# mspaintenjoyer/DepthEstimation

Measured on AMD Instinct MI355X. Metric: disparity Mpix/s at 1080p d_max=128; 1/2/4/8-GPU scaling + %HBM roofline, higher is better.
Workload: dtype u8

## Files before the change

depthestimation_amd/csrc/dsx_bm.hip:

```cpp
#include "dsx_internal.h"
#include "dsx_partition.h"
#include "dsx_subpix.h"

constexpr int kWpe = 3;
constexpr int kWpeSsd = 4;

#ifndef DSX_ROWSTEP_PAIRTAIL
#define DSX_ROWSTEP_PAIRTAIL 0
#endif
#ifndef DSX_ROWSTEP_DIVQ
#define DSX_ROWSTEP_DIVQ 1
#endif
#ifndef DSX_ROWSTEP_OVERLAP
#define DSX_ROWSTEP_OVERLAP 1
#endif
#ifndef DSX_ROWSTEP_AHEAD
#define DSX_ROWSTEP_AHEAD 1
#endif
#ifndef DSX_ROWSTEP_SREF
#define DSX_ROWSTEP_SREF 0
#endif
#ifndef DSX_ROWSTEP_SARGS
#define DSX_ROWSTEP_SARGS DSX_ROWSTEP_SREF
#endif
#ifndef DSX_ROWSTEP_STAGEAHEAD
#define DSX_ROWSTEP_STAGEAHEAD 0
#endif
constexpr bool kRowstepStageahead = DSX_ROWSTEP_STAGEAHEAD;
#ifndef DSX_ROWSTEP_STORELATE
#define DSX_ROWSTEP_STORELATE 1
#endif
constexpr bool kRowstepStorelate = DSX_ROWSTEP_STORELATE;
constexpr bool kRowstepSref = DSX_ROWSTEP_SREF;
constexpr bool kRowstepSargs = DSX_ROWSTEP_SARGS;
constexpr bool kRowstepOverlap = DSX_ROWSTEP_OVERLAP;
constexpr bool kRowstepAhead = DSX_ROWSTEP_AHEAD;
constexpr bool kRowstepPairtail = DSX_ROWSTEP_PAIRTAIL;
constexpr bool kRowstepDivq = DSX_ROWSTEP_DIVQ;
#ifndef DSX_ROWSTEP_ATID
#define DSX_ROWSTEP_ATID 1
#endif
#ifndef DSX_ROWSTEP_KEY2
#define DSX_ROWSTEP_KEY2 1
#endif
#ifndef DSX_ROWSTEP_MERGE
#define DSX_ROWSTEP_MERGE 1
#endif
constexpr bool kRowstepMerge = DSX_ROWSTEP_MERGE;
constexpr bool kRowstepAtid = DSX_ROWSTEP_ATID;
constexpr bool kRowstepKey2 = DSX_ROWSTEP_KEY2;
#ifndef DSX_SEGSTART_AHEAD
#define DSX_SEGSTART_AHEAD 1
#endif
#ifndef DSX_SEGSTART_BATCH
#define DSX_SEGSTART_BATCH 1
#endif
#ifndef DSX_SEGSTART_SPART
#define DSX_SEGSTART_SPART 0
#endif
#ifndef DSX_SEGSTART_ROW0
#define DSX_SEGSTART_ROW0 0
#endif
constexpr bool kSegstartRow0 = DSX_SEGSTART_ROW0;
constexpr bool kSegstartAhead = DSX_SEGSTART_AHEAD;
constexpr bool kSegstartBatch = DSX_SEGSTART_BATCH;
constexpr bool kSegstartSpart = DSX_SEGSTART_SPART;

#include <algorithm>
#include <cstdio>
#include <cstdlib>
#include <cstring>
#include <mutex>
#include <type_traits>
#include <utility>
#include <vector>

namespace dsx {

typedef unsigned short u16x2 __attribute__((ext_vector_type(2)));
typedef uint32_t u32x2 __attribute__((ext_vector_type(2)));
__device__ __forceinline__ u32x2 lds_read_b64(const uint8_t *p) {
    return *(const volatile __attribute__((address_space(3))) u32x2 *)p;
}

__device__ __forceinline__ u16x2 as2(uint32_t v) { return __builtin_bit_cast(u16x2, v); }
__device__ __forceinline__ uint32_t as1(u16x2 v) { return __builtin_bit_cast(uint32_t, v); }
__device__ __forceinline__ int clampi2(int v, int lo, int hi) { return v < lo ? lo : (v > hi ? hi : v); }
__device__ __forceinline__ uint32_t umin2(uint32_t a, uint32_t b) { return a < b ? a : b; }
__device__ __forceinline__ u16x2 add_sub2(u16x2 a, u16x2 p, u16x2 q) { return as2(as1(a) + as1(p) - as1(q)); }
__device__ __forceinline__ int mad_i24(int a, int b, int c) {
    int r;
    asm("v_mad_i32_i24 %0, %1, %2, %3" : "=v"(r) : "v"(a), "v"(b), "v"(c));
    return r;
}
__device__ __forceinline__ uint32_t sad_hi_u8(uint32_t a, uint32_t b, uint32_t c) {
    return __builtin_amdgcn_sad_hi_u8(a, b, c);
}
__device__ __forceinline__ uint32_t min_shr1(uint32_t src, uint32_t key) {
    asm("s_nop 1\n\tv_min_u32_dpp %0, %1, %0 wave_shr:1 row_mask:0xf bank_mask:0xf" : "+v"(key) : "v"(src));
    return key;
}
#pragma clang diagnostic push
#pragma clang diagnostic ignored "-Winline-asm"
template <int OFF0, int STRIDE>
__device__ __forceinline__ void lds_store8_addtid(uint32_t m0base, const uint32_t (&v)[8]) {
    static_assert(OFF0 >= 0 && OFF0 + 7 * STRIDE < 65536, "16-bit offset field");
    asm volatile("s_mov_b32 m0, %8\n\ts_nop 0\n\t"
                 "ds_write_addtid_b32 %0 offset:%9\n\t"
                 "ds_write_addtid_b32 %1 offset:%10\n\t"
                 "ds_write_addtid_b32 %2 offset:%11\n\t"
                 "ds_write_addtid_b32 %3 offset:%12\n\t"
                 "ds_write_addtid_b32 %4 offset:%13\n\t"
                 "ds_write_addtid_b32 %5 offset:%14\n\t"
                 "ds_write_addtid_b32 %6 offset:%15\n\t"
                 "ds_write_addtid_b32 %7 offset:%16"
                 :
                 : "v"(v[0]), "v"(v[1]), "v"(v[2]), "v"(v[3]), "v"(v[4]), "v"(v[5]), "v"(v[6]), "v"(v[7]), "s"(m0base),
                   "n"(OFF0), "n"(OFF0 + STRIDE), "n"(OFF0 + 2 * STRIDE), "n"(OFF0 + 3 * STRIDE), "n"(OFF0 + 4 * STRIDE),
                   "n"(OFF0 + 5 * STRIDE), "n"(OFF0 + 6 * STRIDE), "n"(OFF0 + 7 * STRIDE)
                 : "memory", "m0");
}
#pragma clang diagnostic pop
__device__ __forceinline__ void lds_drain() { asm volatile("s_waitcnt lgkmcnt(0)" ::: "memory"); }
__device__ __forceinline__ uint32_t lds_offset(const uint8_t *p) {
    return (uint32_t)(uintptr_t)(const __attribute__((address_space(3))) uint8_t *)p;
}
__host__ __device__ constexpr int rnd16(int v) { return (v + 15) & ~15; }
template <int R, bool SSD, int NW>
struct Geo {
    static constexpr int TX = 32;
    static constexpr int NC = TX + 2 * R;
    static constexpr int KD = SSD ? 1 : 2;
    static constexpr int LDW = 64 * KD;
    static constexpr int Dp = NW * LDW;
    static constexpr int NT = 64 * NW;
    static constexpr int TPP = NT / TX;
    static constexpr int DSL = Dp / TPP;
    static constexpr int CB = SSD ? 4 : 2;
    static constexpr int PITCH = Dp * CB + 16;
    static constexpr int NJ = NC + Dp;
    static constexpr int REFW = rnd16(NC + 4);
    static constexpr int SROW = rnd16(NJ * 4 + 16);
    static constexpr int MAXJ = (NJ + NT - 1) / NT;
    static constexpr int NB = DSL / 8;
    static constexpr int REFB = rnd16(4 * (NC + 8));
    static constexpr int SLOT = SROW + REFB;
    static constexpr int SMEM0 = 4 * SLOT + TX * PITCH;
    static constexpr int SMEM = SMEM0 > (2 * R + 1) * SLOT ? SMEM0 : (2 * R + 1) * SLOT;
    static constexpr int XRB = 128;
};

#ifdef DSX_STAMPS
#define DSX_STAMP(i)                                                                        \
    do {                                                                                    \
        __builtin_amdgcn_sched_barrier(0);                                                  \
        uint64_t t_;                                                                        \
        asm volatile("s_memtime %0\n\ts_waitcnt lgkmcnt(0)" : "=s"(t_)::"memory");          \
        __builtin_amdgcn_sched_barrier(0);                                                  \
        if ((i) > 0) ph[(i)-1] += t_ - t_prev;                                              \
        t_prev = t_;                                                                        \
    } while (0)
#else
#define DSX_STAMP(i) \
    do {             \
    } while (0)
#endif

__device__ __forceinline__ void lds_barrier() {
    __builtin_amdgcn_fence(__ATOMIC_RELEASE, "workgroup", "local");
    __builtin_amdgcn_s_barrier();
    __builtin_amdgcn_fence(__ATOMIC_ACQUIRE, "workgroup", "local");
}

template <int NW>
__device__ __forceinline__ void block_sync() {
    if constexpr (NW == 1) {
        __builtin_amdgcn_fence(__ATOMIC_ACQ_REL, "wavefront", "local");
    } else {
        lds_barrier();
    }
}

template <int TPP>
__device__ __forceinline__ uint32_t gmin(uint32_t v) {
    if constexpr (TPP > 1) v = umin2(v, (uint32_t)__builtin_amdgcn_update_dpp(0, (int)v, 0xB1, 0xF, 0xF, false));
    if constexpr (TPP > 2) v = umin2(v, (uint32_t)__builtin_amdgcn_update_dpp(0, (int)v, 0x4E, 0xF, 0xF, false));
    if constexpr (TPP > 4) v = umin2(v, (uint32_t)__builtin_amdgcn_ds_swizzle((int)v, 0x101F));
    if constexpr (TPP > 8) v = umin2(v, (uint32_t)__builtin_amdgcn_ds_swizzle((int)v, 0x201F));
    return v;
}


typedef const __attribute__((address_space(4))) uint32_t cu32;
typedef const __attribute__((address_space(1))) uint8_t gu8;
typedef const __attribute__((address_space(1))) uint32_t gu32;
typedef __attribute__((address_space(1))) uint8_t gw8;
typedef __attribute__((address_space(1))) int16_t g16;
typedef __attribute__((address_space(1))) float gf32;

template <bool RELOAD>
__device__ __forceinline__ Bm2Args kargs_row(const Bm2Args &a) {
    if constexpr (RELOAD) {
        typedef __attribute__((address_space(4))) const Bm2Args KArgs;
        KArgs *p = (KArgs *)__builtin_amdgcn_kernarg_segment_ptr();
        asm volatile("" : "+s"(p));
        return *(const Bm2Args *)p;
    } else {
        return a;
    }
}

template <int R, bool SSD, int NW, int SIDE, bool FAST, bool ABS, bool LRFULL>
__device__ __forceinline__ void bm2_segment(const Bm2Args &a_in, uint8_t *smem, int x0, int yb, int ye, long fin, long fout,
                                            bool lr_on, int done0, const int (&pe)[3], int &qcur, int wvu
#ifdef DSX_STAMPS
                                            , uint64_t (&ph)[8], uint64_t &t_prev, uint64_t &nsteps
#endif
) {
    using G = Geo<R, SSD, NW>;
    constexpr int TX = G::TX, NC = G::NC, Dp = G::Dp, NT = G::NT, TPP = G::TPP, DSL = G::DSL, CB = G::CB,
                  PITCH = G::PITCH, NJ = G::NJ, SLOT = G::SLOT, NB = G::NB, NJ4 = (NJ + 3) / 4;
    constexpr int side = SIDE;
    const Bm2Args a = kargs_row<SIDE == 3>(a_in);
    constexpr bool FSS = SSD && !ABS && R <= 5 && (SIDE == 0 || SIDE == 3 || SIDE == 4);
    constexpr bool SGK = SIDE == 4;
    constexpr uint32_t OFF = FSS ? 0x4B000000u : 0u;
    constexpr int CW = (!FSS && (SSD || SIDE == 3)) ? 4 : 8, NCH = (NC + CW - 1) / CW;
    typedef typename std::conditional<FSS, float, typename std::conditional<SSD, uint32_t, u16x2>::type>::type acc_t;
    uint8_t *tile = smem + 4 * SLOT;

    constexpr bool LANE_RB = SSD && !ABS && NW >= 4;
    int ln = 0;
    if constexpr (LANE_RB)
        asm volatile("v_mbcnt_lo_u32_b32 %0, -1, 0\n\tv_mbcnt_hi_u32_b32 %0, -1, %0" : "=v"(ln));
    else
        ln = (int)threadIdx.x & 63;
    const int tid = LANE_RB ? (wvu << 6) + ln : (int)threadIdx.x;
    const int wv = LANE_RB ? wvu : tid >> 6;
    const int H = a.H, W = a.W, m = a.m, D = a.D;
    const int64_t stride = a.stride;
    const int d0 = SSD ? (wv * 64 + ln) : (wv * 128 + 2 * ln);
    const uint32_t padv = a.padv;
    const int PB = side == 1 ? (x0 - R + m) : (x0 - R - m + NC - 1);
    const int sgn = side == 1 ? 1 : -1;

    constexpr int NC4 = (NC + 3) / 4;
    constexpr bool RL2 = !SSD;
    uint32_t ofs_r = (uint32_t)(x0 - R + 4 * min(tid, NC4 - 1));
    uint32_t ofs_s = side == 1 ? (uint32_t)(PB + 4 * min(tid, NJ4 - 1)) : (uint32_t)(PB - 4 * min(tid, NJ4 - 1) - 3);
    constexpr bool MRG = kRowstepMerge && RL2 && FAST && SIDE != 3 && SIDE != 2 && !(SIDE == 4 && R >= 7);
    static_assert(!MRG || NJ4 + NC4 <= NT, "merged staging: a lane per staged dword");
    const bool m_s = tid < NJ4;
    const int m_r = min(tid - NJ4, NC4 - 1);
    const uint8_t *m_base = m_s ? a.src + fin + ofs_s : a.ref + fin + (uint32_t)(x0 - R + 4 * m_r);
    const bool m_dn = m_s && side != 1;
    const uint32_t m_sel0 = m_dn ? 0x0C0C0C03u : 0x0C0C0C00u, m_sel1 = m_dn ? 0x0C0C0C02u : 0x0C0C0C01u,
                   m_sel2 = m_dn ? 0x0C0C0C01u : 0x0C0C0C02u, m_sel3 = m_dn ? 0x0C0C0C00u : 0x0C0C0C03u;
    const uint32_t m_lane = m_s ? (uint32_t)(16 * tid) : (uint32_t)(G::SROW + 16 * m_r);
    auto ldm = [&](int r, uint32_t &w) __attribute__((always_inline)) {
        const int yy = clampi2(r, 0, H - 1);
        long ro = (long)yy * stride;
        asm("" : "+s"(ro));
        w = *reinterpret_cast<const uint32_t *>(m_base + ro);
    };
    auto stm = [&](uint8_t *sp, uint32_t w) __attribute__((always_inline)) {
        if (tid < NJ4 + NC4)
            *reinterpret_cast<uint4 *>(sp) = make_uint4(__builtin_amdgcn_perm(0u, w, m_sel0), __builtin_amdgcn_perm(0u, w, m_sel1),
                                                        __builtin_amdgcn_perm(0u, w, m_sel2), __builtin_amdgcn_perm(0u, w, m_sel3));
    };
    constexpr bool SR0 = kSegstartRow0 && kSegstartBatch && MRG && R <= 4 && (SIDE == 0 || SIDE == 4);
    uint32_t sr_n = 0, sr_o = 0;
    auto ld = [&](int r, uint32_t &w0, uint32_t &w1, uint32_t &w2, uint32_t &w3, uint32_t &rf) __attribute__((always_inline)) {
        const int yy = clampi2(r, 0, H - 1);
        const uint8_t *srow_ = a.src + fin + (long)yy * stride;
        const uint8_t *rrow_ = a.ref + fin + (long)yy * stride;
        if constexpr (RL2) {
            asm("" : "+s"(srow_));
            asm("" : "+s"(rrow_));
        }
        typedef typename std::conditional<RL2, gu8, const uint8_t>::type row8;
        typedef typename std::conditional<RL2, gu32, const uint32_t>::type row32;
        typedef typename std::conditional<RL2, uint32_t, int>::type rix;
        row8 *srow = (row8 *)srow_, *rrow = (row8 *)rrow_;
        const int tr = min(tid, NC4 - 1);
        if constexpr (FAST) {
            if constexpr (RL2) {
                rf = *reinterpret_cast<row32 *>(rrow + ofs_r);
            } else {
                rf = *reinterpret_cast<row32 *>(rrow + x0 - R + 4 * tr);
            }
        } else {
            uint32_t v = 0;
#pragma unroll
            for (int q = 0; q < 4; ++q) v |= (uint32_t)rrow[(rix)clampi2(x0 - R + 4 * tr + q, 0, W - 1)] << (8 * q);
            rf = v;
        }
        if constexpr (FAST) {
            const int tj = min(tid, NJ4 - 1);
            row8 *p;
            if constexpr (RL2) {
                p = srow + ofs_s;
            } else {
                p = side == 1 ? srow + PB + 4 * tj : (SIDE == 3 && NW == 1) ? srow + (PB - 4 * tj - 3) : srow + PB - 4 * tj - 3;
            }
            w0 = *reinterpret_cast<row32 *>(p);
            if constexpr (RL2) w1 = w2 = w3 = 0;
        } else {
            uint32_t v[4];
            int t4 = 4 * tid;
            if constexpr (!SSD && NW == 1 && SIDE == 3)
                asm volatile("" : "+v"(t4));
#pragma unroll
            for (int q = 0; q < 4; ++q) {
                const int j = min(t4 + q, NJ - 1);
                const int pp = PB + sgn * j;
                uint32_t t = srow[(rix)clampi2(pp, 0, W - 1)];
                if constexpr (FSS) t = __float_as_uint((float)t);
                v[q] = t;
            }
            w0 = v[0];
            w1 = v[1];
            w2 = v[2];
            w3 = v[3];
        }
    };
    auto st = [&](int sl, uint32_t w0, uint32_t w1, uint32_t w2, uint32_t w3, uint32_t rf) __attribute__((always_inline)) {
        if (FSS && tid < NC4) {
            *reinterpret_cast<uint4 *>(smem + sl * SLOT + G::SROW + 16 * tid) =
                make_uint4(__float_as_uint((float)(rf & 0xFFu)), __float_as_uint((float)((rf >> 8) & 0xFFu)),
                           __float_as_uint((float)((rf >> 16) & 0xFFu)), __float_as_uint((float)(rf >> 24)));
        } else if (tid < NC4) {
            *reinterpret_cast<uint4 *>(smem + sl * SLOT + G::SROW + 16 * tid) =
                make_uint4(rf & 0xFFu, (rf >> 8) & 0xFFu, (rf >> 16) & 0xFFu, rf >> 24);
        }
        if constexpr (FAST) {
            const uint32_t dw = w0;
            if (side == 1) {
                w0 = dw & 0xFFu; w1 = (dw >> 8) & 0xFFu; w2 = (dw >> 16) & 0xFFu; w3 = dw >> 24;
            } else if constexpr (FSS) {
                w0 = __float_as_uint((float)(dw >> 24)); w1 = __float_as_uint((float)((dw >> 16) & 0xFFu));
                w2 = __float_as_uint((float)((dw >> 8) & 0xFFu)); w3 = __float_as_uint((float)(dw & 0xFFu));
            } else {
                w0 = dw >> 24; w1 = (dw >> 16) & 0xFFu; w2 = (dw >> 8) & 0xFFu; w3 = dw & 0xFFu;
            }
        }
        if (tid < NJ4) *reinterpret_cast<uint4 *>(smem + sl * SLOT + 16 * tid) = make_uint4(w0, w1, w2, w3);
    };
    auto st_at = [&](uint8_t *sp, uint32_t w0, uint32_t w1, uint32_t w2, uint32_t w3, uint32_t rf) __attribute__((always_inline)) {
        if (tid < NC4)
            *reinterpret_cast<uint4 *>(sp + G::SROW) = make_uint4(rf & 0xFFu, (rf >> 8) & 0xFFu, (rf >> 16) & 0xFFu, rf >> 24);
        if constexpr (FAST) {
// ... 174 lines not shown
        uint32_t ae[NC], ao[NC];
#pragma unroll
        for (int c = 0; c < NC; ++c) ae[c] = ao[c] = 0;
        constexpr bool IAH = kSegstartAhead && R <= 5;
        if constexpr (IAH) {
#pragma unroll 1
            for (int g = 0; g < NGR; ++g) {
                uint32_t rv[2][4], p0[2][4], p1[2][4];
                auto ird = [&](auto qc) __attribute__((always_inline)) {
                    constexpr int q = decltype(qc)::value, c0 = 4 * q, t = q & 1;
                    const uint4 rr = *reinterpret_cast<const uint4 *>(smem + NGR * TPG + g * RG + 4 * c0);
                    rv[t][0] = rr.x; rv[t][1] = rr.y; rv[t][2] = rr.z; rv[t][3] = rr.w;
#pragma unroll
                    for (int c = 0; c < 4; ++c) {
                        if (c0 + c < NC) {
                            if constexpr (ABS) {
                                p0[t][c] = *reinterpret_cast<const uint32_t *>(tb + g * TPG + (NC - 1 - c0 - c) * 8);
                            } else {
                                const uint2 pr = *reinterpret_cast<const uint2 *>(tb + g * TPG + (NC - 1 - c0 - c) * 8);
                                p0[t][c] = pr.x;
                                p1[t][c] = pr.y;
                            }
                        }
                    }
                };
                auto isad = [&](auto qc) __attribute__((always_inline)) {
                    constexpr int q = decltype(qc)::value, c0 = 4 * q, t = q & 1;
#pragma unroll
                    for (int c = 0; c < 4; ++c) {
                        if (c0 + c < NC) {
                            ae[c0 + c] = __builtin_amdgcn_sad_u8(rv[t][c], p0[t][c], ae[c0 + c]);
                            if constexpr (!ABS) ao[c0 + c] = __builtin_amdgcn_sad_u8(rv[t][c], p1[t][c], ao[c0 + c]);
                        }
                    }
                };
                auto ichunk = [&](auto qc) __attribute__((always_inline)) {
                    constexpr int q = decltype(qc)::value;
                    if constexpr (q < NC4) {
                        __builtin_amdgcn_sched_barrier(0);
                        if constexpr (q + 1 < NC4) ird(std::integral_constant<int, q + 1>{});
                        __builtin_amdgcn_sched_barrier(0);
                        isad(qc);
                    }
                };
                ird(std::integral_constant<int, 0>{});
                ichunk(std::integral_constant<int, 0>{}); ichunk(std::integral_constant<int, 1>{});
                ichunk(std::integral_constant<int, 2>{}); ichunk(std::integral_constant<int, 3>{});
                ichunk(std::integral_constant<int, 4>{}); ichunk(std::integral_constant<int, 5>{});
                ichunk(std::integral_constant<int, 6>{}); ichunk(std::integral_constant<int, 7>{});
                ichunk(std::integral_constant<int, 8>{}); ichunk(std::integral_constant<int, 9>{});
                ichunk(std::integral_constant<int, 10>{}); ichunk(std::integral_constant<int, 11>{});
                static_assert(NC4 <= 12, "column chunks of the transposed init");
                __builtin_amdgcn_sched_barrier(0);
            }
        } else {
#pragma unroll 1
        for (int g = 0; g < NGR; ++g) {
#pragma unroll
            for (int q = 0; q < NC4; ++q) {
                const int c0 = 4 * q;
                const uint4 rr = *reinterpret_cast<const uint4 *>(smem + NGR * TPG + g * RG + 4 * c0);
                const uint32_t rv[4] = {rr.x, rr.y, rr.z, rr.w};
#pragma unroll
                for (int c = 0; c < 4; ++c) {
                    if (c0 + c < NC) {
                        if constexpr (ABS) {
                            const uint32_t p0 = *reinterpret_cast<const uint32_t *>(tb + g * TPG + (NC - 1 - c0 - c) * 8);
                            ae[c0 + c] = __builtin_amdgcn_sad_u8(rv[c], p0, ae[c0 + c]);
                        } else {
                            const uint2 pr = *reinterpret_cast<const uint2 *>(tb + g * TPG + (NC - 1 - c0 - c) * 8);
                            ae[c0 + c] = __builtin_amdgcn_sad_u8(rv[c], pr.x, ae[c0 + c]);
                            ao[c0 + c] = __builtin_amdgcn_sad_u8(rv[c], pr.y, ao[c0 + c]);
                        }
                    }
                }
            }
        }
        }
#pragma unroll
        for (int c = 0; c < NC; ++c) {
            if constexpr (ABS) cs[c] = ae[c];
            else cs[c] = as2(ae[c] | (ao[c] << 16));
        }
        }

    } else {
    block_sync<NW>();
    {
        constexpr int IG = 3;
#pragma unroll 1
        for (int i0 = 0; i0 <= 2 * R; i0 += IG) {
            uint32_t iw[IG][5];
#pragma unroll
            for (int i = 0; i < IG; ++i)
                if (i0 + i <= 2 * R) ld(yb - R + i0 + i, iw[i][0], iw[i][1], iw[i][2], iw[i][3], iw[i][4]);
#pragma unroll
            for (int i = 0; i < IG; ++i)
                if (i0 + i <= 2 * R) st(i0 + i, iw[i][0], iw[i][1], iw[i][2], iw[i][3], iw[i][4]);
        }
    }
    block_sync<NW>();
#pragma unroll 1
    for (int i = 0; i <= 2 * R; ++i) {
        uint32_t nx = 0;
#pragma unroll
        for (int q = 0; q < NCH; ++q) {
            const int c0 = CW * q;
            uint32_t sw[CW + 1], rw[CW];
            float rf8[8];
            s_chunk(i, c0, sw, nx);
            if constexpr (FSS) ref_chunkf(i, c0, rf8);
            else ref_chunk(i, c0, rw);
#pragma unroll
            for (int c = 0; c < CW; ++c) {
                if (c0 + c < NC) {
                    if constexpr (FSS) {
                        const float t = rf8[c] - __uint_as_float(sw[c]);
                        cs[c0 + c] = __builtin_fmaf(t, t, cs[c0 + c]);
                    } else if constexpr (ABS) {
                        cs[c0 + c] = __builtin_amdgcn_sad_u16(rw[c], sw[c], cs[c0 + c]);
                    } else if constexpr (SSD) {
                        const int t = (int)rw[c] - (int)sw[c];
                        cs[c0 + c] += (uint32_t)__mul24(t, t);
                    } else {
                        cs[c0 + c] = as2(sad_hi_u8(rw[c], pair_e1(sw, c), __builtin_amdgcn_sad_u8(rw[c], pair_e0(sw, c), as1(cs[c0 + c]))));
                    }
                }
            }
            if constexpr (SSD) __builtin_amdgcn_sched_barrier(0);
        }
    }
    }
    block_sync<NW>();

    for (int q = tid; q < TX * (Dp - D); q += NT) {
        const int k = q / (Dp - D), d = D + (q - k * (Dp - D));
        if constexpr (SSD) *reinterpret_cast<uint32_t *>(tile + k * PITCH + d * 4) = padv + OFF;
        else *reinterpret_cast<uint16_t *>(tile + k * PITCH + d * 2) = (uint16_t)padv;
    }
    block_sync<NW>();

    const bool edge = side == 1 && (x0 + m < 0 || x0 + TX - 1 + m + Dp - 1 > W - 1);
    const bool dodd = !SSD && (D & 1);
    const bool lane_writes = d0 < D;

    uint32_t stg = (MRG ? m_lane : (uint32_t)(16 * tid)) + (uint32_t)((2 - (yb & 1) * 2) * SLOT);
    constexpr bool PTAIL = kRowstepPairtail && !SSD && SIDE == 0 && NW == 1;
    constexpr bool DIVQ = kRowstepDivq && !SSD && SIDE == 0;
    uint32_t kp0 = 0, kp1 = 0;
    constexpr bool CUQ = !SSD && SIDE == 0 && NW == 1 && R < 6 && kRowstepKey2 && !PTAIL;
    constexpr bool OVL = kRowstepOverlap && CUQ, AHD = kRowstepAhead && CUQ;
    constexpr bool STA = kRowstepStageahead && OVL;
    constexpr bool STL = kRowstepStorelate && OVL;
    int e_fx = 0;
    float e_pf = 0.0f;
    constexpr int CQ = 4, NQ = (NC + CQ - 1) / CQ;
    constexpr bool SREF = kRowstepSref && CUQ && FAST && OVL && R < 5;
    constexpr bool SRA = kRowstepSargs && CUQ && OVL && R < 5;
    static_assert(!SREF || NQ == NC4, "one reference dword per column chunk");
    uint32_t qn[NC4 + 1] = {}, qo[NC4 + 1] = {}, shn = 0, sho = 0;
    auto sld = [&](int r, uint32_t(&q)[NC4 + 1], uint32_t &sh) __attribute__((always_inline)) {
        const int yy = clampi2(r, 0, H - 1);
        const uintptr_t p = (uintptr_t)(a.ref + fin + (long)yy * stride + (x0 - R));
        typedef const __attribute__((address_space(4))) uint8_t cu8;
        cu8 *b = (cu8 *)(p & ~(uintptr_t)3);
#pragma unroll
        for (int i = 0; i < NC4; ++i) q[i] = *(cu32 *)(b + 4 * i);
        q[NC4] = *(cu32 *)(b + ((((uint32_t)p + 4u * NC4 - 1u) & ~3u) - ((uint32_t)p & ~3u)));
        sh = ((uint32_t)p & 3u) * 8u;
    };
    auto sbyte = [](uint32_t w, int c) __attribute__((always_inline)) -> uint32_t {
        return c == 3 ? w >> 24 : (w >> (8 * c)) & 0xFFu;
    };
    constexpr int RPS = NQ >= 10 ? 1 : 2, NRS = 8 / RPS;
    static_assert(NQ >= NRS + 2, "a column chunk per stage up to the element keys");
    const int ek = tid / TPP, eh = tid % TPP, ex = x0 + ek;
    const uint8_t *epx = tile + ek * PITCH + eh * DSL * CB;
    uint4 etv[2] = {};
    uint32_t ekmin = 0, ecb = 0, egblk = 0, ecm = 0, ecp = 0;
    int eb = 0, ef = 0, eden = 1;
    bool esp = false;
    auto emin8 = [](uint4 v) __attribute__((always_inline)) -> uint32_t {
        const u16x2 mm = __builtin_elementwise_min(__builtin_elementwise_min(as2(v.x), as2(v.y)),
                                                   __builtin_elementwise_min(as2(v.z), as2(v.w)));
        return umin2(mm.x, mm.y);
    };
    auto estore = [&](int ey, const Bm2Args &ea) __attribute__((always_inline)) {
        if (eh == 0 && ex < W) {
            const long o = fout + (long)ey * W + ex;
            if (ea.out_fixed) ea.out_fixed[o] = (int16_t)e_fx;
            if (ea.out_float) ea.out_float[o] = ea.float_mode == 0 ? (float)(int16_t)e_fx * 0.0625f : e_pf;
        }
    };
    auto estage = [&](auto sc, int ey, auto rl, const Bm2Args &er, auto dfr) __attribute__((always_inline)) {
        constexpr int s = decltype(sc)::value;
        constexpr bool RL = decltype(rl)::value;
        constexpr bool DFR = decltype(dfr)::value;
        auto pick = [&]() __attribute__((always_inline)) -> const Bm2Args & {
            if constexpr (RL) return er;
            else return a;
        };
        const Bm2Args &ea = pick();
        static_assert(!OVL || (NB == 8 && TPP == 2), "overlapped epilogue: 64 disparities per lane, two lanes per pixel");
        constexpr int GB = Dp / 8 <= 16 ? 4 : (Dp / 8 <= 32 ? 5 : 6);
        if constexpr (s <= NRS) {
            if constexpr (s == 0) ekmin = 0xFFFFFFFFu;
#pragma unroll
            for (int j = 0; j < (s > 0 ? RPS : 0); ++j) ekmin = umin2(ekmin, (emin8(etv[j]) << GB) | (uint32_t)(RPS * (s - 1) + j));
            if constexpr (s < NRS) {
#pragma unroll
                for (int j = 0; j < RPS; ++j) etv[j] = *reinterpret_cast<const uint4 *>(epx + 16 * (RPS * s + j));
            } else {
                const uint32_t kmin = gmin<TPP>(ekmin | (uint32_t)(eh * 8));
                ecb = kmin >> GB;
                egblk = kmin & ((1u << GB) - 1u);
                etv[0] = *reinterpret_cast<const uint4 *>(epx + 16 * (egblk & 7u));
            }
        } else if constexpr (s == NRS + 1) {
            const uint32_t w4[4] = {etv[0].x, etv[0].y, etv[0].z, etv[0].w};
            uint32_t k8 = 0xFFFFFFFFu;
#pragma unroll
            for (int q = 0; q < 4; ++q) {
                k8 = umin2(k8, (w4[q] << 16) | (uint32_t)(2 * q));
                k8 = umin2(k8, (w4[q] & 0xFFFF0000u) | (uint32_t)(2 * q + 1));
            }
            const uint32_t dl = (int)(egblk / 8) == eh ? egblk * 8 + (k8 & 7u) : 0xFFFFu;
            eb = (int)gmin<TPP>(dl);
            const uint16_t *pc = reinterpret_cast<const uint16_t *>(tile + ek * PITCH) + eb;
            ecm = pc[-1];
            ecp = pc[1];
        } else if constexpr (s == NRS + 2) {
            esp = ea.subpix && eb > 0 && eb < D - 1;
            int32_t den = (int32_t)ecm + (int32_t)ecp - 2 * (int32_t)ecb;
            eden = den < 1 ? 1 : den;
            const int32_t num = ((int32_t)ecm - (int32_t)ecp) * 16 + eden;
            const int32_t q = DIVQ ? subpix_quot(num, 2 * eden) : div_trunc_small(num, 2 * eden);
            ef = eb * 16 + (esp ? q : 0);
        } else {
            const uint32_t padv_e = RL ? er.padv : padv;
// ... 55 lines not shown
    if constexpr (SR0) {
        if (yb + 1 < ye) {
            stm(smem + stg, sr_n);
            stm(smem + stg + SLOT, sr_o);
        }
        stg = (2 * m_lane + (uint32_t)(2 * SLOT)) - stg;
    }
    for (int y = yb; y < ye; ++y) {
        const Bm2Args &a = kargs_row<SIDE == 3>(a_in);
#ifdef DSX_STAMPS
        ++nsteps;
#endif
        DSX_STAMP(0);
        if (a.prio) {
            const int dn = done0 + (y - yb);
            const int q = RL2 ? (int)(((uint32_t)(pe[0] - 1 - dn) >> 31) + ((uint32_t)(pe[1] - 1 - dn) >> 31) +
                                      ((uint32_t)(pe[2] - 1 - dn) >> 31))
                              : (dn >= pe[0]) + (dn >= pe[1]) + (dn >= pe[2]);
            if (q != qcur) {
                qcur = q;
                switch (q) {
                    case 0: __builtin_amdgcn_s_setprio(3); break;
                    case 1: __builtin_amdgcn_s_setprio(2); break;
                    case 2: __builtin_amdgcn_s_setprio(1); break;
                    default: __builtin_amdgcn_s_setprio(0); break;
                }
            }
        }
        if constexpr (RL2 && FAST && !MRG) asm volatile("" : "+v"(ofs_r), "+v"(ofs_s));
        const int par = (y & 1) * 2;
        const bool more = y + 1 < ye;
        uint32_t pn0 = 0, pn1 = 0, pn2 = 0, pn3 = 0, pnr = 0, po0 = 0, po1 = 0, po2 = 0, po3 = 0, por = 0;
        if constexpr (SR0) {
            if (y > yb) {
                ldm(y + 1 + R, pn0);
                ldm(y - R, po0);
            }
        } else if constexpr (MRG) {
            ldm(y + 1 + R, pn0);
            ldm(y - R, po0);
        } else if (RL2 || more) {
            ld(y + 1 + R, pn0, pn1, pn2, pn3, pnr);
            ld(y - R, po0, po1, po2, po3, por);
        }
        if constexpr (FSS) {
          if (y > yb) {
#pragma unroll
            for (int q = 0; q < (NC + 3) / 4; ++q) {
                const int c0 = 4 * q;
                const uint4 rn = *reinterpret_cast<const uint4 *>(smem + par * SLOT + G::SROW + 4 * c0);
                const uint4 ro = *reinterpret_cast<const uint4 *>(smem + (par + 1) * SLOT + G::SROW + 4 * c0);
                const float rn4[4] = {__uint_as_float(rn.x), __uint_as_float(rn.y), __uint_as_float(rn.z), __uint_as_float(rn.w)};
                const float ro4[4] = {__uint_as_float(ro.x), __uint_as_float(ro.y), __uint_as_float(ro.z), __uint_as_float(ro.w)};
                const uint8_t *bn = smem + par * SLOT + d0 * 4, *bo = smem + (par + 1) * SLOT + d0 * 4;
#pragma unroll
                for (int c = 0; c < 4; ++c) {
                    if (c0 + c < NC) {
                        const float sn = *reinterpret_cast<const float *>(bn + (NC - 1 - c0 - c) * 4);
                        const float so = *reinterpret_cast<const float *>(bo + (NC - 1 - c0 - c) * 4);
                        const float tn = rn4[c] - sn, to = ro4[c] - so;
                        cs[c0 + c] = __builtin_fmaf(-to, to, __builtin_fmaf(tn, tn, cs[c0 + c]));
                    }
                }
            }
          }
        } else if constexpr (OVL || AHD) {
          if (y > yb) {
            uint32_t sn[2][CQ + 1], so[2][CQ + 1], rn[2][CQ], ro[2][CQ];
            uint32_t nxn = 0, nxo = 0;
            auto rd = [&](auto qc) __attribute__((always_inline)) {
                constexpr int q = decltype(qc)::value, c0 = CQ * q, t = AHD ? (q & 1) : 0;
                const uint8_t *bn = (const uint8_t *)__builtin_assume_aligned(smem + par * SLOT + d0 * 4, 8);
                const uint8_t *bo = (const uint8_t *)__builtin_assume_aligned(smem + (par + 1) * SLOT + d0 * 4, 8);
                if constexpr (!SREF) {
                    const uint4 vn = *reinterpret_cast<const uint4 *>(smem + par * SLOT + G::SROW + 4 * c0);
                    const uint4 vo = *reinterpret_cast<const uint4 *>(smem + (par + 1) * SLOT + G::SROW + 4 * c0);
                    rn[t][0] = vn.x; rn[t][1] = vn.y; rn[t][2] = vn.z; rn[t][3] = vn.w;
                    ro[t][0] = vo.x; ro[t][1] = vo.y; ro[t][2] = vo.z; ro[t][3] = vo.w;
                }
                sn[t][0] = c0 == 0 ? *reinterpret_cast<const uint32_t *>(bn + NC * 4) : nxn;
                so[t][0] = c0 == 0 ? *reinterpret_cast<const uint32_t *>(bo + NC * 4) : nxo;
#pragma unroll
                for (int c = 1; c < CQ; c += 2) {
                    if (c0 + c < NC) {
                        const u32x2 pn = lds_read_b64(bn + (NC - 1 - c0 - c) * 4);
                        const u32x2 po = lds_read_b64(bo + (NC - 1 - c0 - c) * 4);
                        sn[t][c + 1] = pn.x; sn[t][c] = pn.y; nxn = pn.x;
                        so[t][c + 1] = po.x; so[t][c] = po.y; nxo = po.x;
                    }
                }
            };
            auto sads = [&](auto qc) __attribute__((always_inline)) {
                constexpr int q = decltype(qc)::value, c0 = CQ * q, t = AHD ? (q & 1) : 0;
                uint32_t wn = 0, wo = 0;
                if constexpr (SREF) {
                    uint32_t hn = qn[q + 1], ho = qo[q + 1];
                    asm("" : "+s"(hn));
                    asm("" : "+s"(ho));
                    wn = (uint32_t)((((uint64_t)hn << 32) | qn[q]) >> shn);
                    wo = (uint32_t)((((uint64_t)ho << 32) | qo[q]) >> sho);
                }
#pragma unroll
                for (int c = 0; c < CQ; ++c) {
                    if (c0 + c < NC) {
                        const uint32_t bn = SREF ? sbyte(wn, c) : rn[t][c], bo = SREF ? sbyte(wo, c) : ro[t][c];
                        const uint32_t en = sad_hi_u8(bn, sn[t][c], __builtin_amdgcn_sad_u8(bn, sn[t][c + 1], as1(cs[c0 + c])));
                        const uint32_t lo = sad_hi_u8(bo, so[t][c], __builtin_amdgcn_sad_u8(bo, so[t][c + 1], 0u));
                        uint32_t v = en - lo;
                        if constexpr (OVL) asm volatile("" : "+v"(v));
                        cs[c0 + c] = as2(v);
                    }
                }
            };
            auto chunk = [&](auto qc) __attribute__((always_inline)) {
                constexpr int q = decltype(qc)::value;
                if constexpr (q < NQ) {
                    __builtin_amdgcn_sched_barrier(0);
                    if constexpr (OVL && q < NRS + 3) estage(qc, y - 1, std::false_type{}, a, std::false_type{});
                    if constexpr (!AHD) rd(qc);
                    else if constexpr (q + 1 < NQ) rd(std::integral_constant<int, q + 1>{});
                    __builtin_amdgcn_sched_barrier(0);
                    sads(qc);
                }
            };
            if constexpr (AHD) rd(std::integral_constant<int, 0>{});
            chunk(std::integral_constant<int, 0>{}); chunk(std::integral_constant<int, 1>{});
            chunk(std::integral_constant<int, 2>{}); chunk(std::integral_constant<int, 3>{});
            chunk(std::integral_constant<int, 4>{}); chunk(std::integral_constant<int, 5>{});
            chunk(std::integral_constant<int, 6>{}); chunk(std::integral_constant<int, 7>{});
            chunk(std::integral_constant<int, 8>{}); chunk(std::integral_constant<int, 9>{});
            chunk(std::integral_constant<int, 10>{}); chunk(std::integral_constant<int, 11>{});
            static_assert(NQ <= 12 && NQ >= 7, "chunks of the overlapped column update");
            __builtin_amdgcn_sched_barrier(0);
            if constexpr (STA) {
                if constexpr (MRG) {
                    if (more) {
                        stm(smem + stg, pn0);
                        stm(smem + stg + SLOT, po0);
                    }
                    stg = (2 * m_lane + (uint32_t)(2 * SLOT)) - stg;
                } else {
                    if (more) {
                        st_at(smem + stg, pn0, pn1, pn2, pn3, pnr);
                        st_at(smem + stg + SLOT, po0, po1, po2, po3, por);
                    }
                    stg = (uint32_t)(32 * tid + 2 * SLOT) - stg;
                }
                __builtin_amdgcn_sched_barrier(0);
            }
            if constexpr (SREF) {
                sld(y + 1 + R, qn, shn);
                sld(y - R, qo, sho);
            }
            const Bm2Args &ea = kargs_row<SRA>(a);
            if constexpr (SRA) __builtin_amdgcn_sched_barrier(0);
            if constexpr (OVL) {
                if constexpr (NQ < NRS + 3) estage(std::integral_constant<int, NRS + 2>{}, y - 1, std::integral_constant<bool, SRA>{}, ea, std::false_type{});
                estage(std::integral_constant<int, NRS + 3>{}, y - 1, std::integral_constant<bool, SRA>{}, ea, std::integral_constant<bool, STL>{});
            }
          }
        } else if (y > yb) {
            uint32_t nxn = 0, nxo = 0;
#pragma unroll
            for (int q = 0; q < NCH; ++q) {
                const int c0 = CW * q;
                uint32_t sn[CW + 1], so[CW + 1], rn[CW], ro[CW];
                ref_chunk(par, c0, rn);
                ref_chunk(par + 1, c0, ro);
                s_chunk(par, c0, sn, nxn);
                s_chunk(par + 1, c0, so, nxo);
#pragma unroll
                for (int c = 0; c < CW; ++c) {
                    if (c0 + c < NC) {
                        if constexpr (ABS) {
                            cs[c0 + c] = __builtin_amdgcn_sad_u16(rn[c], sn[c], cs[c0 + c]) -
                                         __builtin_amdgcn_sad_u16(ro[c], so[c], 0u);
                        } else if constexpr (SSD) {
                            const int tn = (int)rn[c] - (int)sn[c];
                            const int to = (int)ro[c] - (int)so[c];
                            const int nto = (int)so[c] - (int)ro[c];
                            cs[c0 + c] = (uint32_t)mad_i24(to, nto, mad_i24(tn, tn, (int)cs[c0 + c]));
                        } else {
                            const uint32_t en = sad_hi_u8(rn[c], pair_e1(sn, c), __builtin_amdgcn_sad_u8(rn[c], pair_e0(sn, c), as1(cs[c0 + c])));
                            const uint32_t lo = sad_hi_u8(ro[c], pair_e1(so, c), __builtin_amdgcn_sad_u8(ro[c], pair_e0(so, c), 0u));
                            cs[c0 + c] = as2(en - lo);
                        }
                    }
                }
            }
        }
        DSX_STAMP(1);
        DSX_STAMP(2);
        {
            uint8_t *tb = tile + d0 * CB;
            constexpr bool ATID = kRowstepAtid && !SSD && SIDE != 3;
            auto abits = [](acc_t v) __attribute__((always_inline)) -> uint32_t {
                if constexpr (FSS) return __float_as_uint(v);
                else if constexpr (SSD) return v;
                else return as1(v);
            };
            acc_t acc = cs[0];
            if constexpr (FSS) acc = 8388608.0f + cs[0];
#pragma unroll
            for (int c = 1; c <= 2 * R; ++c) {
                if constexpr (SSD) acc += cs[c];
                else acc = as2(as1(acc) + as1(cs[c]));
            }
            if constexpr (side == 3) {
                static_assert(SSD || NW <= 4, "SAD exit slots: 16 B of padding per tile row");
                const int ks = a.kshift;
                const uint32_t selE = d0 < D ? 0x05040100u : 0x0D0D0D0Du;
                const uint32_t selO = d0 + 1 < D ? 0x07060100u : 0x0D0D0D0Du;
                const uint32_t dmE = d0 < D ? (uint32_t)d0 : 0xFFFFFFFFu;
                const bool lane0 = ln == 0;
                const bool top = ln == 63;
                constexpr bool XREG = !SSD;
                uint8_t *xq = XREG ? smem + G::SMEM + G::XRB * wv : tile + Dp * CB + 4 * wv;
                constexpr int XST = XREG ? 4 : PITCH;
                uint32_t X[4] = {0xFFFFFFFFu, 0xFFFFFFFFu, 0xFFFFFFFFu, 0xFFFFFFFFu};
                uint32_t Ae = 0xFFFFFFFFu, Ao = 0xFFFFFFFFu, E = 0xFFFFFFFFu;
                auto diag_loop = [&](auto fullc) __attribute__((always_inline)) {
                    constexpr bool FULL = decltype(fullc)::value;
#pragma unroll
                    for (int k = 0; k < TX; ++k) {
                        if (k > 0) {
                            if constexpr (FSS) acc = (acc - cs[k - 1]) + cs[k + 2 * R];
                            else if constexpr (SSD) acc = acc + cs[k + 2 * R] - cs[k - 1];
                            else acc = add_sub2(acc, cs[k + 2 * R], cs[k - 1]);
                        }
                        if (FULL || lane_writes) {
                            if constexpr (SSD) *reinterpret_cast<uint32_t *>(tb + k * PITCH) = abits(acc);
                            else *reinterpret_cast<uint32_t *>(tb + k * PITCH) = as1(acc);
                        }
                        if constexpr (SSD) {
                            if (FULL || x0 + k < W) Ae = umin2(Ae, (abits(acc) << ks) | dmE);
                            if (k < TX - 1) {
                                const uint32_t F = (uint32_t)__builtin_amdgcn_mov_dpp((int)Ae, 0x13C, 0xF, 0xF, false);
                                E = (uint32_t)__builtin_amdgcn_update_dpp((int)F, (int)E, 0x138, 0xF, 0xF, false);
                                Ae = lane0 ? 0xFFFFFFFFu : F;
                            }
                        } else {
                            const uint32_t kE = __builtin_amdgcn_perm(as1(acc), (uint32_t)d0, selE);
                            const uint32_t kO = __builtin_amdgcn_perm(as1(acc), (uint32_t)(d0 + 1), selO);
                            if constexpr (FULL) {
                                if (k > 0) {
                                    const uint32_t nE = min_shr1(Ao, kE);
                                    Ao = umin2(Ae, kO);
                                    Ae = nE;
                                } else {
                                    Ae = kE;
                                    Ao = kO;
                                }
                            } else {
                                if (k > 0) {
                                    const uint32_t sh = (uint32_t)__builtin_amdgcn_update_dpp(-1, (int)Ao, 0x138, 0xF, 0xF, false);
                                    Ao = Ae;
                                    Ae = sh;
                                }
                                if (x0 + k < W) {
                                    Ae = umin2(Ae, kE);
                                    Ao = umin2(Ao, kO);
                                }
                            }
                            if (k < TX - 1) {
                                if constexpr (FULL) {
                                    X[k & 3] = Ao;
                                    if (((k & 3) == 3 || k == TX - 2) && top)
                                        *reinterpret_cast<uint4 *>(xq + (k & ~3) * 4) = make_uint4(X[0], X[1], X[2], X[3]);
                                } else if (top) {
                                    *reinterpret_cast<uint32_t *>(xq + k * XST) = Ao;
                                }
                            }
                        }
                    }
                };
                if constexpr (LRFULL) diag_loop(std::true_type{});
                else diag_loop(std::false_type{});
                uint32_t *krow = a.lr_keys + fout + (long)y * W;
                const int dtop = (wv + 1) * G::LDW - 1;
                if constexpr (SSD) {
                    const int xe = x0 + (TX - 2 - ln) - m - dtop;
                    if (ln < TX - 1 && E != 0xFFFFFFFFu && xe >= 0 && xe < W) atomicMin(krow + xe, E);
                } else if (ln < TX - 1) {
                    E = *reinterpret_cast<const uint32_t *>(xq + ln * XST);
                    const int xe = x0 + ln - m - dtop;
                    if (E != 0xFFFFFFFFu && xe >= 0 && xe < W) atomicMin(krow + xe, E);
                }
                const int xa = x0 + TX - 1 - m - d0;
                if (Ae != 0xFFFFFFFFu && xa >= 0 && xa < W) atomicMin(krow + xa, Ae);
                if constexpr (!SSD) {
                    if (Ao != 0xFFFFFFFFu && xa - 1 >= 0 && xa - 1 < W) atomicMin(krow + xa - 1, Ao);
                }
            } else if (ATID && lane_writes) {
                static_assert(!ATID || (TX % 8 == 0 && G::LDW * CB == 256), "addtid: a lane's tile bytes are 4 * lane");
                if constexpr (ATID) {
                const uint32_t mb = lds_offset(tile) + (uint32_t)wvu * (uint32_t)(G::LDW * CB);
                auto grp = [&](auto k0c) __attribute__((always_inline)) {
                    constexpr int k0 = decltype(k0c)::value;
                    uint32_t v[8];
#pragma unroll
                    for (int j = 0; j < 8; ++j) {
                        if (k0 + j > 0) acc = add_sub2(acc, cs[k0 + j + 2 * R], cs[k0 + j - 1]);
                        v[j] = as1(acc);
                    }
                    lds_store8_addtid<k0 * PITCH, PITCH>(mb, v);
                };
                grp(std::integral_constant<int, 0>{});
                grp(std::integral_constant<int, 8>{});
                grp(std::integral_constant<int, 16>{});
                grp(std::integral_constant<int, 24>{});
                }
            } else if (lane_writes) {
#pragma unroll
                for (int k = 0; k < TX; ++k) {
                    if (k > 0) {
                        if constexpr (FSS) acc = (acc - cs[k - 1]) + cs[k + 2 * R];
                        else if constexpr (SSD) acc = acc + cs[k + 2 * R] - cs[k - 1];
                        else acc = add_sub2(acc, cs[k + 2 * R], cs[k - 1]);
                    }
                    if constexpr (SSD) *reinterpret_cast<uint32_t *>(tb + k * PITCH) = abits(acc);
                    else *reinterpret_cast<uint32_t *>(tb + k * PITCH) = as1(acc);
                }
            }
            if (dodd && d0 + 1 == D) {
                for (int k = 0; k < TX; ++k) *reinterpret_cast<uint16_t *>(tb + k * PITCH + 2) = (uint16_t)padv;
            }
            if (edge && lane_writes) {
                const int base = x0 + m + d0;
                for (int k = 0; k < TX; ++k) {
                    const int p0 = base + k;
                    if constexpr (SSD) {
                        if (p0 < 0 || p0 > W - 1) *reinterpret_cast<uint32_t *>(tb + k * PITCH) = padv;
                    } else {
                        if (p0 < 0 || p0 > W - 1) *reinterpret_cast<uint16_t *>(tb + k * PITCH) = (uint16_t)padv;
                        if (p0 + 1 < 0 || p0 + 1 > W - 1) *reinterpret_cast<uint16_t *>(tb + k * PITCH + 2) = (uint16_t)padv;
                    }
                }
            }
        }
        DSX_STAMP(3);
        if constexpr (kRowstepAtid && !SSD && SIDE != 3 && NW > 1) lds_drain();
        block_sync<NW>();
        DSX_STAMP(4);
        if constexpr (RL2) {
            [[maybe_unused]] const bool late = STA ? (!SR0 && y == yb) : (!SR0 || y > yb);
            if constexpr (MRG) {
                if (more && late) {
                    stm(smem + stg, pn0);
                    stm(smem + stg + SLOT, po0);
                }
                if (late) stg = (2 * m_lane + (uint32_t)(2 * SLOT)) - stg;
            } else if constexpr (SIDE != 3) {
                if (more && late) {
                    st_at(smem + stg, pn0, pn1, pn2, pn3, pnr);
                    st_at(smem + stg + SLOT, po0, po1, po2, po3, por);
                }
                if (late) stg = (uint32_t)(32 * tid + 2 * SLOT) - stg;
            } else if (more) {
                st(par ^ 2, pn0, pn1, pn2, pn3, pnr);
                st((par ^ 2) + 1, po0, po1, po2, po3, por);
            }
        }
        if constexpr (STL) {
            if (y > yb) estore(y - 1, a);
        }
        DSX_STAMP(5);
        if constexpr (side == 2) {
            constexpr int CPP = Dp * CB / 16;
            for (int q = tid; q < TX * CPP; q += NT) {
                const int k = q / CPP, off = (q - k * CPP) * 16;
                const int x = x0 + k;
                if (x < W) {
                    const uint4 v = *reinterpret_cast<const uint4 *>(tile + k * PITCH + off);
                    *reinterpret_cast<uint4 *>(reinterpret_cast<uint8_t *>(a.vol) + ((size_t)fout + (size_t)y * W + x) * (Dp * CB) + off) = v;
                }
            }
        } else if constexpr (!OVL) {
            const int k = tid / TPP, h = tid % TPP;
            const int x = x0 + k;
            const uint8_t *px = tile + k * PITCH + h * DSL * CB;
            uint32_t bs[NB];
#pragma unroll
            for (int i = 0; i < NB; ++i) {
                if constexpr (SSD) {
                    const uint4 v0 = *reinterpret_cast<const uint4 *>(px + 32 * i);
                    const uint4 v1 = *reinterpret_cast<const uint4 *>(px + 32 * i + 16);
// ... 530 lines not shown
```

Before: 48070.

## Store 3-column group sums so box filter uses add3 instead of sliding window

```diff
diff --git a/depthestimation_amd/csrc/dsx_bm.hip b/depthestimation_amd/csrc/dsx_bm.hip
--- a/depthestimation_amd/csrc/dsx_bm.hip
+++ b/depthestimation_amd/csrc/dsx_bm.hip
@@ -47,6 +47,10 @@
 #define DSX_ROWSTEP_MERGE 1
 #endif
 constexpr bool kRowstepMerge = DSX_ROWSTEP_MERGE;
+#ifndef DSX_ROWSTEP_COLGROUP
+#define DSX_ROWSTEP_COLGROUP 1
+#endif
+constexpr bool kRowstepColgroup = DSX_ROWSTEP_COLGROUP;
 constexpr bool kRowstepAtid = DSX_ROWSTEP_ATID;
 constexpr bool kRowstepKey2 = DSX_ROWSTEP_KEY2;
 #ifndef DSX_SEGSTART_AHEAD
@@ -91,6 +95,11 @@
 __device__ __forceinline__ int mad_i24(int a, int b, int c) {
     int r;
     asm("v_mad_i32_i24 %0, %1, %2, %3" : "=v"(r) : "v"(a), "v"(b), "v"(c));
+    return r;
+}
+__device__ __forceinline__ uint32_t add3_u32(uint32_t a, uint32_t b, uint32_t c) {
+    uint32_t r;
+    asm("v_add3_u32 %0, %1, %2, %3" : "=v"(r) : "v"(a), "v"(b), "v"(c));
     return r;
 }
 __device__ __forceinline__ uint32_t sad_hi_u8(uint32_t a, uint32_t b, uint32_t c) {
@@ -130,6 +139,7 @@
 struct Geo {
     static constexpr int TX = 32;
     static constexpr int NC = TX + 2 * R;
+    static constexpr int NG3 = NC - 2;
     static constexpr int KD = SSD ? 1 : 2;
     static constexpr int LDW = 64 * KD;
     static constexpr int Dp = NW * LDW;
@@ -250,12 +260,17 @@
     uint32_t ofs_s = side == 1 ? (uint32_t)(PB + 4 * min(tid, NJ4 - 1)) : (uint32_t)(PB - 4 * min(tid, NJ4 - 1) - 3);
     constexpr bool MRG = kRowstepMerge && RL2 && FAST && SIDE != 3 && SIDE != 2 && !(SIDE == 4 && R >= 7);
     static_assert(!MRG || NJ4 + NC4 <= NT, "merged staging: a lane per staged dword");
+    constexpr bool CG = kRowstepColgroup && MRG && SIDE == 0 && NW == 1 && (R == 4 || R == 1) && kRowstepKey2 &&
+                        !kRowstepPairtail && kRowstepOverlap && kRowstepAhead && !kRowstepSref;
+    constexpr int NCU = CG ? G::NG3 : NC;
     const bool m_s = tid < NJ4;
-    const int m_r = min(tid - NJ4, NC4 - 1);
+    const int m_r = CG ? max(NC4 - 1 - (tid - NJ4), 0) : min(tid - NJ4, NC4 - 1);
     const uint8_t *m_base = m_s ? a.src + fin + ofs_s : a.ref + fin + (uint32_t)(x0 - R + 4 * m_r);
     const bool m_dn = m_s && side != 1;
-    const uint32_t m_sel0 = m_dn ? 0x0C0C0C03u : 0x0C0C0C00u, m_sel1 = m_dn ? 0x0C0C0C02u : 0x0C0C0C01u,
-                   m_sel2 = m_dn ? 0x0C0C0C01u : 0x0C0C0C02u, m_sel3 = m_dn ? 0x0C0C0C00u : 0x0C0C0C03u;
+    const uint32_t m_sel0 = CG ? (m_dn ? 0x0C050403u : 0x0C020100u) : (m_dn ? 0x0C0C0C03u : 0x0C0C0C00u),
+                   m_sel1 = CG ? (m_dn ? 0x0C040302u : 0x0C030201u) : (m_dn ? 0x0C0C0C02u : 0x0C0C0C01u),
+                   m_sel2 = CG ? (m_dn ? 0x0C030201u : 0x0C040302u) : (m_dn ? 0x0C0C0C01u : 0x0C0C0C02u),
+                   m_sel3 = CG ? (m_dn ? 0x0C020100u : 0x0C050403u) : (m_dn ? 0x0C0C0C00u : 0x0C0C0C03u);
     const uint32_t m_lane = m_s ? (uint32_t)(16 * tid) : (uint32_t)(G::SROW + 16 * m_r);
     auto ldm = [&](int r, uint32_t &w) __attribute__((always_inline)) {
         const int yy = clampi2(r, 0, H - 1);
@@ -264,9 +279,10 @@
         w = *reinterpret_cast<const uint32_t *>(m_base + ro);
     };
     auto stm = [&](uint8_t *sp, uint32_t w) __attribute__((always_inline)) {
+        const uint32_t nb = CG ? (uint32_t)__builtin_amdgcn_mov_dpp((int)w, 0x138, 0xF, 0xF, true) : 0u;
         if (tid < NJ4 + NC4)
-            *reinterpret_cast<uint4 *>(sp) = make_uint4(__builtin_amdgcn_perm(0u, w, m_sel0), __builtin_amdgcn_perm(0u, w, m_sel1),
-                                                        __builtin_amdgcn_perm(0u, w, m_sel2), __builtin_amdgcn_perm(0u, w, m_sel3));
+            *reinterpret_cast<uint4 *>(sp) = make_uint4(__builtin_amdgcn_perm(nb, w, m_sel0), __builtin_amdgcn_perm(nb, w, m_sel1),
+                                                        __builtin_amdgcn_perm(nb, w, m_sel2), __builtin_amdgcn_perm(nb, w, m_sel3));
     };
     constexpr bool SR0 = kSegstartRow0 && kSegstartBatch && MRG && R <= 4 && (SIDE == 0 || SIDE == 4);
     uint32_t sr_n = 0, sr_o = 0;
@@ -607,6 +623,10 @@
             if constexpr (ABS) cs[c] = ae[c];
             else cs[c] = as2(ae[c] | (ao[c] << 16));
         }
+        if constexpr (CG) {
+#pragma unroll
+            for (int c = 0; c < G::NG3; ++c) cs[c] = as2(as1(cs[c]) + as1(cs[c + 1]) + as1(cs[c + 2]));
+        }
         }
 
     } else {
@@ -679,7 +699,8 @@
     constexpr bool STL = kRowstepStorelate && OVL;
     int e_fx = 0;
     float e_pf = 0.0f;
-    constexpr int CQ = 4, NQ = (NC + CQ - 1) / CQ;
+    static_assert(!CG || (CUQ && OVL && AHD), "group sums: the rotated loop with its reads ahead");
+    constexpr int CQ = 4, NQ = (NCU + CQ - 1) / CQ;
     constexpr bool SREF = kRowstepSref && CUQ && FAST && OVL && R < 5;
     constexpr bool SRA = kRowstepSargs && CUQ && OVL && R < 5;
     static_assert(!SREF || NQ == NC4, "one reference dword per column chunk");
@@ -901,7 +922,7 @@
                 so[t][0] = c0 == 0 ? *reinterpret_cast<const uint32_t *>(bo + NC * 4) : nxo;
 #pragma unroll
                 for (int c = 1; c < CQ; c += 2) {
-                    if (c0 + c < NC) {
+                    if (c0 + c < NCU) {
                         const u32x2 pn = lds_read_b64(bn + (NC - 1 - c0 - c) * 4);
                         const u32x2 po = lds_read_b64(bo + (NC - 1 - c0 - c) * 4);
                         sn[t][c + 1] = pn.x; sn[t][c] = pn.y; nxn = pn.x;
@@ -921,7 +942,7 @@
                 }
 #pragma unroll
                 for (int c = 0; c < CQ; ++c) {
-                    if (c0 + c < NC) {
+                    if (c0 + c < NCU) {
                         const uint32_t bn = SREF ? sbyte(wn, c) : rn[t][c], bo = SREF ? sbyte(wo, c) : ro[t][c];
                         const uint32_t en = sad_hi_u8(bn, sn[t][c], __builtin_amdgcn_sad_u8(bn, sn[t][c + 1], as1(cs[c0 + c])));
                         const uint32_t lo = sad_hi_u8(bo, so[t][c], __builtin_amdgcn_sad_u8(bo, so[t][c + 1], 0u));
@@ -1020,10 +1041,12 @@
             };
             acc_t acc = cs[0];
             if constexpr (FSS) acc = 8388608.0f + cs[0];
+            if constexpr (!CG) {
 #pragma unroll
             for (int c = 1; c <= 2 * R; ++c) {
                 if constexpr (SSD) acc += cs[c];
                 else acc = as2(as1(acc) + as1(cs[c]));
+            }
             }
             if constexpr (side == 3) {
                 static_assert(SSD || NW <= 4, "SAD exit slots: 16 B of padding per tile row");
@@ -1119,8 +1142,12 @@
                     uint32_t v[8];
 #pragma unroll
                     for (int j = 0; j < 8; ++j) {
-                        if (k0 + j > 0) acc = add_sub2(acc, cs[k0 + j + 2 * R], cs[k0 + j - 1]);
-                        v[j] = as1(acc);
+                        if constexpr (CG) {
+                            v[j] = R == 4 ? add3_u32(as1(cs[k0 + j]), as1(cs[k0 + j + 3]), as1(cs[k0 + j + 6])) : as1(cs[k0 + j]);
+                        } else {
+                            if (k0 + j > 0) acc = add_sub2(acc, cs[k0 + j + 2 * R], cs[k0 + j - 1]);
+                            v[j] = as1(acc);
+                        }
                     }
                     lds_store8_addtid<k0 * PITCH, PITCH>(mb, v);
                 };
```

Result: faster. 49860 (median of 6 runs) (+3.7%).
